# zloyaloha/ray-tracing-practice

Measured on AMD Instinct MI355X. Metric: Msamples/sec (pixels x spp / s), path-traced frame, higher is better.
Workload: dtype f32

## Files before the change

### include/rtp_amd.h

```cpp
#ifndef RTP_AMD_H
#define RTP_AMD_H

#include <stdint.h>

#ifdef __cplusplus
extern "C" {
#endif

typedef enum rt_status {
    RT_OK = 0,
    RT_ERR_INVALID_ARG = 1,
    RT_ERR_NO_DEVICE = 2,
    RT_ERR_HIP = 3,
    RT_ERR_UNSUPPORTED = 4,
    RT_ERR_OUT_OF_MEMORY = 5
} rt_status;


typedef struct rt_vec3 { float e[3]; } rt_vec3;

typedef struct rt_sphere {
    rt_vec3 center;
    float   radius;
    int32_t material_idx;
// ... 107 lines not shown
    int32_t  guard_repack;
    int32_t  kernel;
    uint64_t workspace_bytes;
    int32_t  pass_spp;
    int32_t  stack_levels;
    uint32_t flag_capacity;
    int32_t  scene_in_lds;
    int32_t  lds_treelet;
    int32_t  workgroups_per_cu;
    int32_t  k_inner, k_shade;
    int32_t  reserve_chunk;
    int32_t  reserve_taper;
    int32_t  wavefront_paths;
    int32_t  wavefront_exchange;
    int32_t  wide_nodes;
    int32_t  guard_dynamic_margins;
    int32_t  sphere_only_kernel;
    int32_t  overlap_rework;
    int32_t  primary_visibility;
    int32_t  guard_bail_share;
    int32_t  guard_front_primitives;
    int32_t  reuse_view_lists;
    int32_t  resume_flagged;
} rt_config;


rt_status rt_set_device(int32_t device_ordinal);

rt_status rt_scene_create(const rt_scene_desc *desc, rt_scene **out_scene);

void rt_config_init_sized(rt_config *cfg, uint32_t struct_bytes);
void rt_config_init(rt_config *cfg);
#define rt_config_init(cfg) rt_config_init_sized((cfg), (uint32_t)sizeof(rt_config))
void rt_config_from_env(rt_config *cfg);
rt_status rt_scene_create_ex(const rt_scene_desc *desc, const rt_config *cfg, rt_scene **out_scene);
rt_status rt_scene_set_config(rt_scene *scene, const rt_config *cfg);
rt_status rt_scene_get_config(const rt_scene *scene, rt_config *cfg);

rt_status rt_scene_destroy(rt_scene *scene);

const char *rt_scene_guard_reason(const rt_scene *scene);

int32_t rt_shard_rows(int32_t image_height, const rt_shard *shard);

rt_status rt_render(rt_scene *scene, const rt_camera_data *cam, const rt_shard *shard,
                    float *d_fb_sum, void *hip_stream, int32_t sync, rt_timing *timing);
// ... 144 lines not shown
```

### ray-tracing-practice_amd/csrc/rt_accel.cpp

```cpp
#include "rt_accel.h"
#include "rt_device_math.h"

#include <algorithm>
#include <cmath>
#include <cstdlib>
#include <cstring>
#include <functional>

namespace rtaccel {
namespace {

inline float bits_as_float(int32_t v) { float f; std::memcpy(&f, &v, 4); return f; }

struct LeafRef {
    float box[6];
    int32_t code;
};

struct BuildNode {
    float box[6];
    int32_t child[2];
};

void box_union(const float a[6], const float b[6], float out[6]) {
// ... 479 lines not shown
            out.leaf_boxes.assign(static_cast<size_t>(d.num_spheres) * 8, 0.0f);
            out.plane_leaf_boxes.assign(static_cast<size_t>(d.num_planes) * 8, 0.0f);
            for (LeafRef &l : leaves) {
                const int32_t code = -(l.code + 1);
                const int32_t i = code >> 1;
                float *lb = (code & 1) ? &out.plane_leaf_boxes[static_cast<size_t>(i) * 8] : &out.leaf_boxes[static_cast<size_t>(i) * 8];
                for (int a = 0; a < 6; ++a) lb[a] = l.box[a];
                const double e = (code & 1) ? eps_plane : std::max(eps[static_cast<size_t>(i)], eps_floor);
                const float ef = static_cast<float>(e * (1.0 + 1e-6));
                for (int a = 0; a < 3; ++a) {
                    l.box[2 * a] = std::nextafterf(l.box[2 * a] - ef, -INFINITY);
                    l.box[2 * a + 1] = std::nextafterf(l.box[2 * a + 1] + ef, INFINITY);
                }
            }
            bool derivable = true;
            for (int i = 0; i < d.num_spheres && derivable; ++i) {
                if (leaf_of_sphere[static_cast<size_t>(i)] < 0) continue;
                const rt_sphere &s = d.spheres[i];
                const float *lb = &out.leaf_boxes[static_cast<size_t>(i) * 8];
                for (int a = 0; a < 3; ++a)
                    if (lb[2 * a] != s.center.e[a] - s.radius || lb[2 * a + 1] != s.center.e[a] + s.radius) derivable = false;
            }
            if (derivable && !opt.leaf_table) out.leaf_boxes.clear();
            g.ok = why.empty();
            g.num_front = 0;
            const int front_max = std::min(opt.front_max, kMaxFront);
            while (g.ok && g.num_front < front_max && leaves.size() > 2) {
                float all[6] = {INFINITY, -INFINITY, INFINITY, -INFINITY, INFINITY, -INFINITY};
                size_t big = 0;
                for (size_t k = 0; k < leaves.size(); ++k) {
                    box_union(all, leaves[k].box, all);
                    if (half_area(leaves[k].box) > half_area(leaves[big].box)) big = k;
                }
                if (!(half_area(leaves[big].box) >= 0.5f * half_area(all))) break;
                g.front_code[g.num_front] = -(leaves[big].code + 1);
                std::memcpy(g.front_box[g.num_front], leaves[big].box, sizeof(float) * 6);
                g.num_front++;
                leaves.erase(leaves.begin() + static_cast<std::ptrdiff_t>(big));
            }
            for (int a = 1; a < g.num_front; ++a)
                for (int b = a; b > 0 && (g.front_code[b] & 1) && !(g.front_code[b - 1] & 1); --b) {
                    std::swap(g.front_code[b], g.front_code[b - 1]);
                    for (int k = 0; k < 6; ++k) std::swap(g.front_box[b][k], g.front_box[b - 1][k]);
                }
        }
        g.reason = why;
// ... 315 lines not shown
```

### ray-tracing-practice_amd/csrc/rt_accel.h

```cpp
#pragma once
#include <cstdint>
#include <string>
#include <vector>
#include "../../include/rtp_amd.h"

namespace rtaccel {

constexpr int32_t kTraversalDone = INT32_MIN;

inline int32_t leaf_code(int32_t prim_index, int32_t prim_type) { return -(2 * prim_index + prim_type) - 1; }

constexpr int kMaxFront = 4;

struct Packed {
    std::vector<float> nodes;
    std::vector<float> hnodes;
    std::vector<float> spheres;
    std::vector<int32_t> sphere_mat;
    std::vector<float> planes;
    std::vector<float> materials;
    std::vector<float> tex_data;
    std::vector<int32_t> tex_info;
    std::vector<float> tnodes;
    int32_t num_tnodes = 0;
// ... 3 lines not shown
    int32_t num_internal = 0;
    bool full_pairs = true;
    int32_t num_top_pairs = 0;
    int32_t max_depth = 0;
    std::vector<float> wnodes;
    std::vector<float> whnodes;
    int32_t num_wide = 0, num_top_wide = 0, wroot = kTraversalDone, wide_depth = 0;
    struct Guard {
        bool ok = false;
        std::string reason;
        float center[3] = {0, 0, 0};
        float d0_sq = 0;
        float cluster_radius = 0;
        float box[6] = {0, 0, 0, 0, 0, 0};
        float far_k = 0;
        float dyn_k = 0;
        float dyn_rmax = 0;
        int32_t num_small = 0, num_large = 0;
        float origin_center[3] = {0, 0, 0};
        float origin_radius = 0;
        int32_t num_front = 0;
        int32_t front_code[kMaxFront] = {0, 0, 0, 0};
        float front_box[kMaxFront][6] = {};
    } guard;
    std::vector<float> leaf_boxes;
    std::vector<float> plane_leaf_boxes;
    std::vector<float> guard_leaf_boxes;
    std::vector<int32_t> guard_leaf_codes;
};

enum class TreeMode { Reference, Sah, Guarded, GuardedLeaves };

constexpr float kGuardGammaBound = 24.0f * 5.9604645e-8f;
constexpr float kGuardGammaObserved = 8.0f * 5.9604645e-8f;

struct PackOptions {
    double gamma = kGuardGammaBound;
    bool leaf_table = false;
    int dynamic = 0;
    int front_max = kMaxFront;
    int lds_pair_budget = 0;
};

float half_to_float(uint16_t h);
uint16_t float_to_half_dir(float f, bool toward_minus_inf);

std::string pack_scene(const rt_scene_desc &desc, TreeMode mode, Packed &out, const PackOptions &opt = PackOptions(),
                       const float *camera_hint = nullptr);


struct Magic { uint32_t m, s; };
bool make_magic(uint32_t d, uint64_t n_max, Magic &g);

constexpr uint64_t kWorkIndexLimit = (uint64_t)1 << 30;
constexpr uint64_t kWorkIndexMargin = 64;
constexpr uint64_t kMaxCallPixels = (uint64_t)1 << 24;
constexpr int kMaxPasses = 1024;
constexpr uint64_t kSampleBytes = 12;
constexpr uint64_t kWorkspaceShareOfDevice = 16;

// ... 11 lines not shown
```

### ray-tracing-practice_amd/csrc/rt_capi.hip

```cpp
#include <hip/hip_runtime.h>

#include <cmath>
#include <cstdio>
#include <cstdlib>
#include <cstring>
#include <new>
#include <string>
#include <vector>

#include "../../include/rtp_amd.h"
#include "rt_accel.h"
#include "rt_build.h"
#include "rt_device_math.h"
#include "rt_kernel.hip.inc"
#include "rt_primary.hip.inc"
#include "rt_aov.hip.inc"
#include "rt_adaptive.hip.inc"
#include "rt_nee.hip.inc"
#include "rt_env.hip.inc"
#include "rt_light.hip.inc"

namespace {

thread_local std::string g_last_error;
// ... 47 lines not shown
bool guarded_wanted(const rt_config &cfg, int64_t primitives) {
    if (cfg.traversal == RT_TRAVERSAL_GUARDED) return true;
    return primitives >= cfg.guard_min_primitives;
}

void config_defaults(rt_config &c) {
    std::memset(&c, 0, sizeof(c));
    c.struct_bytes = (uint32_t)sizeof(rt_config);
    c.tree_build = RT_BUILD_HOST_SAH;
    c.guard_gamma_ulps = 0.0f;
    c.traversal = RT_TRAVERSAL_AUTO;
    c.guard_min_primitives = 64;
    c.guard_repack = 1;
    c.kernel = RT_KERNEL_AUTO;
    c.workspace_bytes = 0;
    c.scene_in_lds = 1;
    c.lds_treelet = 1;
    c.reserve_taper = 1;
    c.wide_nodes = 0;
    c.guard_bail_share = 0;
    c.guard_front_primitives = 0;
    c.reuse_view_lists = 0;
    c.resume_flagged = 0;
}

rt_config config_from_caller(const rt_config *in) {
    rt_config c;
    config_defaults(c);
    if (in && in->struct_bytes >= 8) {
        const size_t n = in->struct_bytes < sizeof(rt_config) ? in->struct_bytes : sizeof(rt_config);
        std::memcpy(&c, in, n);
        c.struct_bytes = (uint32_t)sizeof(rt_config);
    }
    if (c.guard_min_primitives < 0) c.guard_min_primitives = 0;
    return c;
}

int32_t lds_pair_budget(const rt_scene_desc &d) {
    bool plain = d.num_planes == 0;
    for (int i = 0; plain && i < d.num_materials; ++i) plain = d.materials[i].texture_id == 0;
    const int64_t budget = (int64_t)kLdsLimit / 2;
    const int64_t lanes = plain ? rtk::kSimpleBlock : rtk::kBlock;
    const int64_t fixed = (int64_t)d.num_spheres * 16 + ((int64_t)d.num_spheres + 3) / 4 * 16 + (int64_t)d.num_planes * 80 +
                          (plain ? 0 : (int64_t)d.num_materials * 16 * RTP_LDS_MAT_ROWS) + 16 * rtk::kConstRows + (lanes / 64) * (8 + 32 * 4) + 7 * lanes * 4;
    const int64_t nodes = (budget - fixed) / rtk::kOctNodeBytes;
    return (int32_t)(nodes < 1 ? 1 : nodes);
}

rtaccel::PackOptions pack_options(const rt_config &cfg, const rt_scene_desc *d = nullptr) {
    rtaccel::PackOptions o;
    if (d && cfg.scene_in_lds != 0) o.lds_pair_budget = lds_pair_budget(*d);
    o.dynamic = cfg.guard_dynamic_margins;
    if (cfg.guard_gamma_ulps > 0.0f) o.gamma = (double)cfg.guard_gamma_ulps * 5.9604644775390625e-8;
    o.leaf_table = cfg.guard_exact_leaf_table != 0;
    o.front_max = cfg.guard_front_primitives < 0 ? 0 : rtaccel::kMaxFront;
    return o;
}
uint32_t bail_share_of(const rt_config &cfg) {
    if (cfg.guard_bail_share < 0) return 0u;
    const uint32_t s = cfg.guard_bail_share == 0 ? kDefaultBailShare : (uint32_t)cfg.guard_bail_share;
    return s > 255u ? 255u : s;
}
uint32_t bail_floor() {
    static const uint32_t f = [] { const int v = env_int("RTP_BAIL_FLOOR", (int)kDefaultBailFloor); return (uint32_t)(v < 0 ? 0 : v > 255 ? 255 : v); }();
    return f;
}
uint32_t bail_latest() {
    static const uint32_t f = [] { const int v = env_int("RTP_BAIL_LATEST", (int)kDefaultBailLatest); return (uint32_t)(v < 1 ? 1 : v > 8 ? 8 : v); }();
    return f;
}
template <class T>
void copy_out(const T &src, T *dst, uint32_t caller_bytes) {
    const uint32_t n = caller_bytes < sizeof(T) ? caller_bytes : (uint32_t)sizeof(T);
    std::memcpy(dst, &src, n);
    dst->struct_bytes = n;
}
rt_status timing_check(const rt_timing *t) {
    if (t && t->struct_bytes < 8) { g_last_error = "rt_timing.struct_bytes is not set (rt_timing_init)"; return RT_ERR_INVALID_ARG; }
// ... 50 lines not shown
    int4 *tex_info = nullptr;
    uint32_t *queue = nullptr;
    float *slab = nullptr;
    size_t slab_floats = 0;
    rtaccel::Packed::Guard guard;
    std::vector<rt_sphere> host_spheres;
    std::vector<rt_plane> host_planes;
    std::vector<rt_bvh_node> host_nodes;
    bool device_built = false;
    int repacks = 0;
    bool repack_refused = false;
    bool guard_paused = false;
    struct Feedback {
        uint32_t *host = nullptr; hipEvent_t start = nullptr, done = nullptr;
        bool pending = false, guarded = false, exploring = false;
        int passes = 0; uint64_t samples = 0, serial = 0;
    };
    Feedback feedback[kFeedbackSlots];
    int feedback_next = 0;
    double guarded_ns_per_sample = 0.0, exact_ns_per_sample = 0.0;
    bool explore_exact = false;
    uint64_t frame_serial = 0;
    uint32_t trip_test = 0;
    const uint32_t *last_traced_pixels = nullptr;
    int32_t last_spp = 0;
    float4 *leaf_boxes = nullptr, *plane_leaf_boxes = nullptr;
    uint32_t *flag_list = nullptr;
    uint32_t *resume_tag = nullptr; float4 *resume_state = nullptr;
    size_t flag_cap = 0;
    uint32_t *dirty = nullptr, *dirty_list = nullptr;
    size_t dirty_cap = 0;
    hipStream_t aux_stream = nullptr, list_stream = nullptr;
    hipEvent_t ev_fork = nullptr, ev_join = nullptr, ev_listed = nullptr;
    uint32_t *cand = nullptr;
    size_t cand_pixels = 0;
    struct CandKey { float view[12]; int32_t dims[9]; int repacks; hipStream_t stream; bool valid = false; } cand_key;
    int32_t num_internal = 0, num_spheres = 0, num_planes = 0, num_materials = 0, root = rtk::kDone, tree_depth = 0;
    CallClock clock[kNumClocks];
    std::vector<hipEvent_t> pass_events;
    int timed_passes = 0;
    rt_timing last{};
    int last_passes = 0;
    uint64_t last_samples = 0;
    bool timed = false;
    int num_cus = 0;
    uint64_t device_bytes = 0;
// ... 70 lines not shown
        if (shard && shard->num_parts > 1) return fail(RT_ERR_INVALID_ARG, "a tile and a shard in one call");
        if (tile->w <= 0 || tile->h <= 0 || tile->x0 < 0 || tile->y0 < 0 || (int64_t)tile->x0 + tile->w > cam->image_width ||
            (int64_t)tile->y0 + tile->h > cam->image_height)
            return fail(RT_ERR_INVALID_ARG, "tile outside the image");
        P.local_rows = tile->h;
        P.row_w = tile->w;
        P.tile_x0 = tile->x0;
        P.tile_y0 = tile->y0;
    }
    P.nodes = sc->nodes; P.hnodes = sc->hnodes; P.num_internal = sc->num_internal; P.root = sc->root;
    P.whnodes = sc->whnodes; P.wroot = sc->wroot;
    P.tnodes = sc->tnodes; P.num_tnodes = sc->num_tnodes;
    P.xnodes = sc->xnodes; P.num_top = sc->num_top;
    P.spheres = sc->spheres; P.num_spheres = sc->num_spheres;
    P.planes = sc->planes; P.num_planes = sc->num_planes;
    P.materials = sc->materials; P.num_materials = sc->num_materials;
    P.sphere_mat = sc->sphere_mat;
    P.tex_data = sc->tex_data; P.tex_info = sc->tex_info;
    P.queue = sc->queue;
    if ((uint64_t)P.local_rows * (uint64_t)P.row_w > (1u << 24)) return fail(RT_ERR_UNSUPPORTED, "more than 2^24 pixels per call");
    P.total_work = 0;
    P.stats = sc->queue + kQueueStats;
    P.trip_test = sc->trip_test;
    {
        const uint64_t pixels = (uint64_t)P.local_rows * (uint64_t)P.row_w;
        if (!make_magic((uint32_t)P.row_w, pixels + 1, P.magic_width) ||
            !make_magic((uint32_t)P.band_rows, (uint64_t)P.local_rows + 1, P.magic_band))
            return fail(RT_ERR_UNSUPPORTED, "image too large for the work index arithmetic");
    }
    P.stack_levels = 0;
    P.leaf_boxes = sc->leaf_boxes;
    P.plane_leaf_boxes = sc->plane_leaf_boxes;
    std::memcpy(P.g_center, sc->guard.center, 12);
    P.g_d0sq = sc->guard.d0_sq;
    P.g_rs = sc->guard.cluster_radius;
    P.g_fark = sc->guard.far_k;
    P.g_dynk = sc->guard.dyn_k;
    {
        const double sk = std::sqrt((double)sc->guard.dyn_k * (double)rtk::kDynSlack) * (1.0 + 4e-6);
        P.g_dyn_sqrtk = std::nextafterf((float)sk, INFINITY);
        P.g_dyn_b = std::nextafterf((float)(sk * 1.7320508075688772 * (double)sc->guard.dyn_rmax * (1.0 + 1e-6)), INFINITY);
        P.g_dyn_c3 = std::nextafterf((float)(sk * 1.7320508075688772), INFINITY);
        P.g_dyn_kslack = std::nextafterf((float)((double)sc->guard.dyn_k * (double)rtk::kDynSlack), INFINITY);
    }
    P.num_front = sc->guard.num_front;
    std::memcpy(P.front_code, sc->guard.front_code, sizeof(P.front_code));
    std::memcpy(P.front_box, sc->guard.front_box, sizeof(P.front_box));
    std::memcpy(P.g_box, sc->guard.box, 24);
    P.k_inner = sc->cfg.k_inner > 0 ? sc->cfg.k_inner : 24;
    P.k_shade = sc->cfg.k_shade > 0 ? sc->cfg.k_shade : 48;
    P.chunk = 64u;
    return RT_OK;
}

rt_status repack_for_camera(rt_scene *sc, const float cam[3], hipStream_t stream) {
// ... 93 lines not shown
    cfg->guard_keep = env_int("RTP_GUARD_KEEP", cfg->guard_keep);
    if (env_int("RTP_NO_REPACK", 0)) cfg->guard_repack = 0;
    if (const char *v = getenv("RTP_SLAB_GIB")) { const double g = atof(v); if (g > 0) cfg->workspace_bytes = (uint64_t)(g * 1073741824.0); }
    cfg->pass_spp = env_int("RTP_PASS_SPP", cfg->pass_spp);
    cfg->stack_levels = env_int("RTP_STACK_LEVELS", cfg->stack_levels);
    cfg->flag_capacity = (uint32_t)env_int("RTP_FLAG_CAP", (int)cfg->flag_capacity);
    if (env_int("RTP_NO_LDS_SCENE", 0)) cfg->scene_in_lds = 0;
    if (env_int("RTP_NO_TREELET", 0)) cfg->lds_treelet = 0;
    cfg->workgroups_per_cu = env_int("RTP_WGS_PER_CU", cfg->workgroups_per_cu);
    cfg->k_inner = env_int("RTP_K_INNER", cfg->k_inner);
    cfg->k_shade = env_int("RTP_K_SHADE", cfg->k_shade);
    cfg->reserve_chunk = env_int("RTP_CHUNK", cfg->reserve_chunk);
    cfg->wavefront_paths = env_int("RTP_WF_PATHS", cfg->wavefront_paths);
    cfg->wavefront_exchange = env_int("RTP_WF_EXCHANGE", cfg->wavefront_exchange);
    if (env_int("RTP_NO_TAPER", 0)) cfg->reserve_taper = 0;
    cfg->wide_nodes = env_int("RTP_WIDE", cfg->wide_nodes);
    if (env_int("RTP_NO_SIMPLE", 0)) cfg->sphere_only_kernel = -1;
    if (env_int("RTP_NO_OVERLAP", 0)) cfg->overlap_rework = -1;
    if (env_int("RTP_NO_PRIMARY", 0)) cfg->primary_visibility = -1;
    cfg->guard_bail_share = env_int("RTP_BAIL_SHARE", cfg->guard_bail_share);
    if (env_int("RTP_NO_FRONT", 0)) cfg->guard_front_primitives = -1;
    if (env_int("RTP_NO_VIEW_CACHE", 0)) cfg->reuse_view_lists = -1;
    if (env_int("RTP_NO_RESUME", 0)) cfg->resume_flagged = -1;
    copy_out(full, user, user->struct_bytes);
}

rt_status rt_scene_create(const rt_scene_desc *desc, rt_scene **out_scene) { return rt_scene_create_ex(desc, nullptr, out_scene); }

rt_status rt_scene_set_config(rt_scene *sc, const rt_config *cfg) {
    if (!sc || !cfg) return fail(RT_ERR_INVALID_ARG, "null argument");
    rt_config c = config_from_caller(cfg);
    c.tree_build = sc->cfg.tree_build;
    c.guard_gamma_ulps = sc->cfg.guard_gamma_ulps;
    c.guard_exact_leaf_table = sc->cfg.guard_exact_leaf_table;
    c.guard_dynamic_margins = sc->cfg.guard_dynamic_margins;
    c.guard_front_primitives = sc->cfg.guard_front_primitives;
    sc->cfg = c;
    return RT_OK;
}

rt_status rt_scene_get_config(const rt_scene *sc, rt_config *cfg) {
    if (!sc || !cfg) return fail(RT_ERR_INVALID_ARG, "null argument");
    if (cfg->struct_bytes < 8) return fail(RT_ERR_INVALID_ARG, "rt_config.struct_bytes is not set (rt_config_init)");
    copy_out(sc->cfg, cfg, cfg->struct_bytes);
    return RT_OK;
}

rt_status rt_scene_create_ex(const rt_scene_desc *desc, const rt_config *user_cfg, rt_scene **out_scene) {
    if (!desc || !out_scene) return fail(RT_ERR_INVALID_ARG, "null argument");
    *out_scene = nullptr;
    const rt_config cfg = config_from_caller(user_cfg);
    if (cfg.guard_gamma_ulps < 0.0f || !(cfg.guard_gamma_ulps == cfg.guard_gamma_ulps)) return fail(RT_ERR_INVALID_ARG, "guard_gamma_ulps must be >= 0");
    rtaccel::Packed pk;
    const rtaccel::PackOptions popt = pack_options(cfg, desc);
    const bool device_build = cfg.tree_build == RT_BUILD_DEVICE_LBVH;
    std::string err = rtaccel::pack_scene(*desc, device_build ? rtaccel::TreeMode::GuardedLeaves : rtaccel::TreeMode::Guarded, pk, popt);
    if (!err.empty()) return fail(RT_ERR_INVALID_ARG, err);
    if (device_build && !pk.guard.ok) {
        err = rtaccel::pack_scene(*desc, rtaccel::TreeMode::Guarded, pk, popt);
// ... 52 lines not shown
        sc->host_nodes.assign(desc->nodes, desc->nodes + desc->num_nodes);
        sc->device_built = device_build;
    }
    if (hipMalloc((void **)&sc->queue, kQueueWords * 4) != hipSuccess) return bail(fail(RT_ERR_OUT_OF_MEMORY, "hipMalloc(queue) failed"));
    if (sc->clock[kClockRender].make() != RT_OK) return bail(fail(RT_ERR_HIP, "hipEventCreate failed"));
    sc->num_internal = pk.num_internal;
    sc->num_top_pairs = pk.num_top_pairs;
    sc->num_spheres = (int32_t)pk.sphere_mat.size();
    sc->num_planes = (int32_t)(pk.planes.size() / 20);
    sc->num_materials = (int32_t)(pk.materials.size() / 12);
    sc->root = pk.root;
    sc->tree_depth = pk.max_depth;
    *out_scene = sc;
    return RT_OK;
}

rt_status rt_scene_destroy(rt_scene *sc) {
    if (!sc) return RT_OK;
    (void)hipFree(sc->tnodes);
    (void)hipFree(sc->xnodes);
    (void)hipFree(sc->nodes); (void)hipFree(sc->hnodes); (void)hipFree(sc->whnodes);
    (void)hipFree(sc->spheres); (void)hipFree(sc->planes); (void)hipFree(sc->materials);
    (void)hipFree(sc->sphere_mat); (void)hipFree(sc->tex_data); (void)hipFree(sc->tex_info); (void)hipFree(sc->queue); (void)hipFree(sc->slab);
    (void)hipFree(sc->leaf_boxes); (void)hipFree(sc->plane_leaf_boxes); (void)hipFree(sc->flag_list);
    (void)hipFree(sc->dirty); (void)hipFree(sc->dirty_list); (void)hipFree(sc->cand);
    (void)hipFree(sc->resume_tag); (void)hipFree(sc->resume_state);
    if (sc->aux_stream) (void)hipStreamDestroy(sc->aux_stream);
    if (sc->list_stream) (void)hipStreamDestroy(sc->list_stream);
    if (sc->ev_listed) (void)hipEventDestroy(sc->ev_listed);
    if (sc->ev_fork) (void)hipEventDestroy(sc->ev_fork);
    if (sc->ev_join) (void)hipEventDestroy(sc->ev_join);
    for (hipEvent_t e : sc->pass_events) (void)hipEventDestroy(e);
    for (hipEvent_t e : sc->aov_events) (void)hipEventDestroy(e);
    for (CallClock &c : sc->clock) c.destroy();
    (void)hipFree(sc->adapt_mom); (void)hipFree(sc->adapt_list); (void)hipFree(sc->adapt_work); (void)hipFree(sc->adapt_counters);
    (void)hipFree(sc->nee_index_dev); (void)hipFree(sc->nee_cdf_dev); (void)hipFree(sc->nee_pmf_dev);
    for (rt_scene::Feedback &f : sc->feedback) {
        if (f.done) { if (f.pending) (void)hipEventSynchronize(f.done); (void)hipEventDestroy(f.done); }
        if (f.start) (void)hipEventDestroy(f.start);
        if (f.host) (void)hipHostFree(f.host);
    }
    delete sc;
    return RT_OK;
}

const char *rt_scene_guard_reason(const rt_scene *sc) {
    if (!sc) return "null scene";
// ... 1746 lines not shown
    const std::string err = rtbuild::build_lbvh(boxes, codes, n, tree);
    if (!err.empty()) return fail(RT_ERR_HIP, "device BVH build: " + err);
    info[0] = tree.root; info[1] = tree.num_internal; info[2] = tree.depth; info[3] = 0;
    hipError_t e = hipSuccess;
    if (tree.num_internal < 0 || tree.num_internal > n - 1) {
        (void)hipFree(tree.nodes); (void)hipFree(tree.hnodes);
        return fail(RT_ERR_HIP, "device BVH build: " + std::to_string(tree.num_internal) + " records for " + std::to_string(n) + " leaves");
    }
    if (tree.num_internal > 0) {
        e = hipMemcpy(nodes_out, tree.nodes, 64 * (size_t)tree.num_internal, hipMemcpyDeviceToHost);
        if (e == hipSuccess) e = hipMemcpy(hnodes_out, tree.hnodes, 32 * (size_t)tree.num_internal, hipMemcpyDeviceToHost);
    }
    (void)hipFree(tree.nodes); (void)hipFree(tree.hnodes);
    HIP_TRY(e);
    return RT_OK;
}

rt_status rt_debug_trip_test(rt_scene *sc, uint32_t on) {
    if (!sc) return fail(RT_ERR_INVALID_ARG, "null argument");
    sc->trip_test = on;
    return RT_OK;
}

rt_status rt_debug_read_stats(rt_scene *sc, uint32_t out[16]) {
    if (!sc || !out) return fail(RT_ERR_INVALID_ARG, "null argument");
    HIP_TRY(hipDeviceSynchronize());
    HIP_TRY(hipMemcpy(out, sc->queue + kQueueStats, 60, hipMemcpyDeviceToHost));
    return RT_OK;
}

#endif

rt_status rt_last_kernel_ms(rt_scene *sc, float *ms) {
    if (!sc || !ms) return fail(RT_ERR_INVALID_ARG, "null argument");
    *ms = 0.0f;
    if (!sc->timed) return RT_OK;
    return sc->clock[kClockRender].elapsed(*ms);
}

rt_status rt_render_to_host(rt_scene *sc, const rt_camera_data *cam, const rt_shard *shard, float *h_fb_sum, rt_timing *timing) {
    if (!sc || !cam || !h_fb_sum) return fail(RT_ERR_INVALID_ARG, "null argument");
    const int32_t rows = rt_shard_rows(cam->image_height, shard);
    const size_t bytes = (size_t)rows * (size_t)(cam->image_width > 0 ? cam->image_width : 0) * 3 * sizeof(float);
    if (bytes == 0) return RT_OK;
    float *d_fb = nullptr;
    Scratch mem;
// ... 97 lines not shown
```

### ray-tracing-practice_amd/csrc/rt_kernel.hip.inc

```
#pragma once

namespace rtk {

using namespace rtd;

constexpr int kWave = 64;
constexpr int32_t kDone = INT32_MIN;
#ifndef RTP_BLOCK
#define RTP_BLOCK 768
#endif
#ifndef RTP_MIN_WAVES
#define RTP_MIN_WAVES 6
#endif
#ifndef RTP_UNROLL
#define RTP_UNROLL 4
#endif
#ifndef RTP_LDS_MAT_ROWS
#define RTP_LDS_MAT_ROWS 1
#endif
#ifndef RTP_UNROLL_WIDE
#define RTP_UNROLL_WIDE 3
#endif
#ifndef RTP_TRIPWIRE
#ifdef RTP_DEV_BUILD
// ... 27 lines not shown
    int32_t row_w, tile_x0, tile_y0;
    const float4 *nodes;     int32_t num_internal; int32_t root;
    const float4 *hnodes;
    const float4 *whnodes;   int32_t wroot;
    const float4 *tnodes;    int32_t num_tnodes;
    const float4 *xnodes;    int32_t num_top;
    const float4 *spheres;   int32_t num_spheres;
    const float4 *planes;    int32_t num_planes;
    const float4 *materials; int32_t num_materials;
    const int32_t *sphere_mat;
    const float4 *tex_data;  const int4 *tex_info;
    float *fb;
    float *slab;
    uint32_t slab_pitch;
    uint32_t num_pixels;
    int32_t pass_first, pass_count;
    Magic magic_count, magic_width, magic_band;
    uint32_t *queue;
    uint32_t chunk;
    uint32_t taper_shift;
    uint32_t full_chunk, full_taper;
    uint32_t *stats;
    uint32_t trip_test;
    uint32_t total_work;
    int32_t stack_levels;
    int32_t k_inner, k_shade;
    const float4 *leaf_boxes;
    const float4 *plane_leaf_boxes;
    float g_center[3]; float g_d0sq, g_rs, g_fark; float g_box[6];
    float g_dynk;
    float g_dyn_sqrtk, g_dyn_b;
    float g_dyn_c3, g_dyn_kslack;
    int32_t num_front; int32_t front_code[4]; float front_box[4 * 6];
    uint32_t *flag_list; uint32_t *flag_count; uint32_t flag_cap;
    uint32_t *abandon; uint32_t bail_share; uint32_t bail_floor, bail_latest;
    uint32_t flag_chunk_words;
    uint32_t *resume_tag; float4 *resume_state; uint32_t resume_shift;
    uint32_t *dirty; uint32_t *dirty_list; uint32_t *dirty_count;
    const uint32_t *work_list; const uint32_t *work_count; uint32_t work_cap;
    uint32_t consts[14 * 4];
    const uint32_t *cand;
    const uint32_t *order;
    const uint32_t *traced_pixels;
    const int32_t *probe_ijs; float *probe_rad; int32_t *probe_rays; uint32_t *probe_seed; int32_t probe_n;
};

struct Lane {
    f3 o, d, inv;
    float closest;
    int32_t hit;
    int32_t node;
    int32_t sp;
    int32_t pend;
    float e;
    uint32_t seed;
    f3 beta, color;
    int32_t depth;
};

__device__ __forceinline__ f3 ld3(const float *p) { return mk(p[0], p[1], p[2]); }
__device__ __forceinline__ int32_t as_int(float f) { return __float_as_int(f); }

template <bool kClamp = false>
__device__ __forceinline__ void begin_ray(Lane &L, f3 o, f3 d, int32_t root) {
    L.o = o;
    L.d = d;
#if RTP_FAST_RCP_SQRT && defined(__HIP_DEVICE_COMPILE__)
    L.inv = mk(recip_estimate(d.x), recip_estimate(d.y), recip_estimate(d.z));
    if (__builtin_expect(!(recip_in_fence(d.x) && recip_in_fence(d.y) && recip_in_fence(d.z)), 0)) L.inv = mk(1.0f / d.x, 1.0f / d.y, 1.0f / d.z);
#else
    L.inv = mk(1.0f / d.x, 1.0f / d.y, 1.0f / d.z);
#endif
    if (kClamp) L.inv = mk(__builtin_amdgcn_fmed3f(L.inv.x, -1e18f, 1e18f), __builtin_amdgcn_fmed3f(L.inv.y, -1e18f, 1e18f), __builtin_amdgcn_fmed3f(L.inv.z, -1e18f, 1e18f));
    L.closest = 1e30f;
    L.hit = -1;
    L.node = root;
    L.sp = 0;
    L.pend = 0;
}

constexpr int32_t kLevelBytes = kWave * 4;
template <bool kSent = false>
__device__ __forceinline__ void pop(Lane &L, const uint32_t *stack) {
    if (kSent) {
        L.sp -= kLevelBytes;
        L.node = (int32_t)*reinterpret_cast<const uint32_t *>(reinterpret_cast<const char *>(stack) + L.sp);
    } else if (L.sp > 0) {
        L.sp--;
        L.node = (int32_t)stack[L.sp * kWave];
    } else {
        L.node = kDone;
    }
}

__device__ __forceinline__ f3 inv_exact(const Lane &L) {
// ... 515 lines not shown
    const float4 t00 = d[y0w * W + x0w], t10 = d[y0w * W + x1], t01 = d[y1 * W + x0w], t11 = d[y1 * W + x1];
    const f3 top = add(scale(1.0f - dx, mk(t00.x, t00.y, t00.z)), scale(dx, mk(t10.x, t10.y, t10.z)));
    const f3 bot = add(scale(1.0f - dx, mk(t01.x, t01.y, t01.z)), scale(dx, mk(t11.x, t11.y, t11.z)));
    return add(scale(1.0f - dy, top), scale(dy, bot));
}

template <bool kSimple = false, bool kClamped = false, class SphereTab>
__device__ __forceinline__ bool guard_final_check(const Lane &L, const KParams &P, SphereTab spheres) {
    const int32_t code = L.hit;
    const int32_t idx = code >> 1;
    float enter;
    bool in;
    if (!kSimple && ((code & 1) || P.leaf_boxes)) {
        const float4 *tab = (code & 1) ? P.plane_leaf_boxes : P.leaf_boxes;
        const float4 B0 = tab[2 * idx], B1 = tab[2 * idx + 1];
        in = slab<kClamped>(L, B0.x, B0.z, B1.x, B0.y, B0.w, B1.y, 1e30f, enter);
    } else {
        const float4 sp = spheres[idx];
        in = slab<kClamped>(L, sp.x - sp.w, sp.y - sp.w, sp.z - sp.w, sp.x + sp.w, sp.y + sp.w, sp.z + sp.w, 1e30f, enter);
    }
    return in && (L.closest > enter);
}

__device__ __forceinline__ f3 scatter_diffuse_dir(f3 in_sphere, f3 normal) {
    const f3 u = unit(in_sphere);
    f3 dir = dot(u, normal) > 0.0f ? u : neg(u);
    if (near_zero(dir)) dir = normal;
    return dir;
}

template <bool kGuard = false, int kMatStride = 3, bool kSimple = false, bool kPrim = false, bool kClamped = false, class SphereTab, class PlaneTab, class MatTab, class IdxTab>
__device__ __forceinline__ bool shade(Lane &L, const KParams &P, SphereTab spheres, PlaneTab planes, MatTab materials,
                                      IdxTab sphere_mat, f3 &out_o, f3 &out_d) {
    if (kGuard && (L.depth & kFlagBit)) return false;
    if (L.hit < 0) {
        L.color = add(L.color, mul(L.beta, mk(P.bg[0], P.bg[1], P.bg[2])));
        return false;
    }
    const int32_t code = L.hit;
    const int32_t idx = code >> 1;
    const float t = L.closest;
    const bool checked = kPrim && (L.depth & kFreshBit) != 0;
    if (kPrim) L.depth &= ~kFreshBit;
    if (kGuard && !(checked | guard_final_check<kSimple, kClamped>(L, P, spheres))) {
        L.depth |= kFlagBit | RTP_WHY(2);
        return false;
    }
    const f3 point = add(L.o, scale(t, L.d));
    f3 normal;
    bool front;
    int32_t mat_idx;
    float tu = 0.0f, tv = 0.0f;
    const bool is_plane = !kSimple && (code & 1) != 0;
    f3 outward = mk(0, 0, 0);
    if (is_plane) {
        const float4 P0 = planes[5 * idx + 0];
        const float4 P2 = planes[5 * idx + 2];
        outward = mk(P0.x, P0.y, P0.z);
        mat_idx = as_int(P2.w);
    } else {
        const float4 s = spheres[idx];
        outward = divs(sub(point, mk(s.x, s.y, s.z)), s.w);
        mat_idx = sphere_mat[idx];
    }
    front = dot(L.d, outward) < 0;
    normal = front ? outward : neg(outward);

    const float4 MA = materials[kMatStride * mat_idx + 0];
    const float4 ME = kMatStride >= 2 ? materials[kMatStride * mat_idx + 1] : P.materials[3 * mat_idx + 1];
    const int32_t type = as_int(MA.w) & 3;
    const int32_t tex_id = kSimple ? 0 : (as_int(MA.w) >> 2);
    f3 albedo = mk(MA.x, MA.y, MA.z);
    if (tex_id != 0) {
        if (is_plane) {
            const float4 P1 = planes[5 * idx + 1];
            const float4 P2 = planes[5 * idx + 2];
            const float4 P3 = planes[5 * idx + 3];
            const float4 P4 = planes[5 * idx + 4];
            const f3 ph = sub(point, mk(P4.x, P4.y, P4.z));
            const f3 w = mk(P1.x, P1.y, P1.z);
            tu = dot(w, cross(ph, mk(P3.x, P3.y, P3.z)));
            tv = dot(w, cross(mk(P2.x, P2.y, P2.z), ph));
        } else {
            const float theta = acos_libm(outward.y);
// ... 647 lines not shown
```

### ray-tracing-practice_amd/csrc/rt_primary.hip.inc

```
#pragma once
#include "rt_beam.h"

namespace rtk {

constexpr int kCandWords = 16;
constexpr uint32_t kCandNone = 0xffffffffu;

__global__ void __launch_bounds__(256) cand_kernel(const KParams P, uint32_t *cand, double coord_max) {
    const uint32_t q = blockIdx.x * 256u + threadIdx.x;
    if (q >= P.num_pixels) return;
    const uint32_t pjl = q / (uint32_t)P.row_w;
    const int32_t pi = (int32_t)(q - pjl * (uint32_t)P.row_w) + P.tile_x0;
    int32_t pj = (int32_t)pjl + P.tile_y0;
    if (P.num_parts != 1) {
        const uint32_t band = pjl / (uint32_t)P.band_rows;
        pj = (int32_t)((band * (uint32_t)P.num_parts + (uint32_t)P.part) * (uint32_t)P.band_rows + (pjl - band * (uint32_t)P.band_rows));
    }
    const rtbeam::Beam beam = rtbeam::make_beam(P.origin, P.p00, P.du, P.dv, pi, pj, coord_max);
    uint32_t codes[kCandWords - 1];
    const float *tab = reinterpret_cast<const float *>(P.nodes);
    int n = rtbeam::beam_candidates(beam, [tab](int32_t k) { return tab + (size_t)k * 16; }, P.root, (double)P.g_dynk, codes, kCandWords - 1);
    n = rtbeam::beam_front_candidates(beam, P.num_front, P.front_code, P.front_box, (double)P.g_dynk, codes, n, kCandWords - 1);
    uint32_t *out = cand + (size_t)q * kCandWords;
    out[0] = n < 0 ? kCandNone : (uint32_t)n;
// ... 100 lines not shown
    return L.hit >= 0 ? L.hit : kPrimMiss;
}
template <bool kPlanes>
__device__ __forceinline__ int32_t test_lane_list(Lane &L, const KParams &P, uint32_t q, float4 &hs) {
    const uint32_t *list = P.cand + (size_t)q * kCandWords;
    const uint32_t n = list[0];
    if (n == kCandNone) return kPrimWalk;
    const RayConst rc = ray_const(L);
    for (uint32_t c = 0; c < n; ++c) {
        const uint32_t code = list[1 + c];
        const int32_t idx = (int32_t)(code >> 1);
        if (kPlanes && (code & 1u)) test_plane<true>(L, P.planes, idx, (int32_t)code);
        else {
            const float4 sp = P.spheres[idx];
            test_sphere_ray<true, true>(L, sp, (int32_t)code, rc.a, rc.da, rc.y);
            if (L.hit == (int32_t)code) hs = sp;
        }
    }
    return L.hit >= 0 ? L.hit : kPrimMiss;
}
template <bool kPlanes>
__device__ __forceinline__ void finish_primary(Lane &L, const KParams &P, int32_t code_out, uint32_t seed1, float4 hs, float *rec) {
    if (P.leaf_boxes == nullptr) {
        float enter;
        const bool in = slab(L, hs.x - hs.w, hs.y - hs.w, hs.z - hs.w, hs.x + hs.w, hs.y + hs.w, hs.z + hs.w, 1e30f, enter);
        const bool sphere_hit = code_out >= 0 && (!kPlanes || !(code_out & 1));
        if (sphere_hit && !(in && L.closest > enter)) L.depth |= kFlagBit;
        if (kPlanes && code_out >= 0 && (code_out & 1) && !guard_final_check<false>(L, P, P.spheres)) L.depth |= kFlagBit;
    } else if (code_out >= 0 && !guard_final_check<false>(L, P, P.spheres)) {
        L.depth |= kFlagBit;
    }
    if (L.depth & kFlagBit) code_out = kPrimFlag;
    rec[0] = L.closest;
    rec[1] = __int_as_float(code_out);
    rec[2] = __uint_as_float(seed1);
}

template <bool kPlanes>
__global__ void __launch_bounds__(256) primary_kernel(const KParams P) {
    const uint32_t lane = threadIdx.x & 63u;
    const uint32_t wave = (blockIdx.x * 256u + threadIdx.x) >> 6, num_waves = gridDim.x * 4u;
    const uint32_t batches = (P.total_work + 63u) >> 6;
    for (uint32_t b = wave; b < batches; b += num_waves) {
        const uint32_t w = b * 64u + lane;
        if (w >= P.total_work) continue;
        int32_t pi, pj;
        uint32_t k, record;
        map_work<false>(P, w, pi, pj, k, 0u, nullptr, nullptr, &record);
        const uint32_t q = P.pass_count == 64 ? (w >> 6) : div_magic(w, P.magic_count);
        if (P.cand[(size_t)q * kCandWords] == 0u) continue;
        Lane L;
        f3 ray_o, ray_d;
        const uint32_t seed1 = sample_seed1(wang_hash((uint32_t)pi * (uint32_t)P.width + (uint32_t)pj), P.pass_first + (int32_t)k);
        camera_ray<false>(L, P, pi, pj, seed1, ray_o, ray_d);
        begin_ray(L, ray_o, ray_d, 0);
        const uint32_t q0 = __builtin_amdgcn_readfirstlane(q);
        float4 hs = make_float4(0.0f, 0.0f, 0.0f, 0.0f);
        const int32_t code_out = __ballot(q != q0) == 0ull ? test_uniform_list<kPlanes>(L, P, q0, hs) : test_lane_list<kPlanes>(L, P, q, hs);
        finish_primary<kPlanes>(L, P, code_out, seed1, hs, P.slab + (size_t)record * 3);
    }
}

template <bool kPlanes>
__global__ void __launch_bounds__(256) primary_pixel_kernel(const KParams P) {
    const uint32_t lane = threadIdx.x & 63u;
    const uint32_t wave = __builtin_amdgcn_readfirstlane((blockIdx.x * 256u + threadIdx.x) >> 6), num_waves = gridDim.x * 4u;
    for (uint32_t q = wave; q < P.num_pixels; q += num_waves) {
        const uint32_t pjl = div_magic(q, P.magic_width);
        const int32_t pi = (int32_t)(q - pjl * (uint32_t)P.row_w) + P.tile_x0;
        int32_t pj = (int32_t)pjl + P.tile_y0;
        if (P.num_parts != 1) {
            const uint32_t band = div_magic(pjl, P.magic_band);
            pj = (int32_t)((band * (uint32_t)P.num_parts + (uint32_t)P.part) * (uint32_t)P.band_rows + (pjl - band * (uint32_t)P.band_rows));
        }
        float *row = P.slab + (size_t)q * P.slab_pitch * 3;
        if (*(k_u32 *)(uintptr_t)(P.cand + (size_t)q * kCandWords) == 0u) continue;
        const uint32_t base_seed = wang_hash((uint32_t)pi * (uint32_t)P.width + (uint32_t)pj);
        for (uint32_t k = lane; k < (uint32_t)P.pass_count; k += 64u) {
            Lane L;
            f3 ray_o, ray_d;
            const uint32_t seed1 = sample_seed1(base_seed, P.pass_first + (int32_t)k);
            camera_ray<false>(L, P, pi, pj, seed1, ray_o, ray_d);
            begin_ray(L, ray_o, ray_d, 0);
            float4 hs = make_float4(0.0f, 0.0f, 0.0f, 0.0f);
            const int32_t code_out = test_uniform_list<kPlanes>(L, P, q, hs);
            finish_primary<kPlanes>(L, P, code_out, seed1, hs, row + (size_t)k * 3);
        }
    }
}

}
```

### ray-tracing-practice_amd/rtp_bindings.py

```python
import ctypes as C
import os

import numpy as np

_HERE = os.path.dirname(os.path.abspath(__file__))


class Vec3(C.Structure):
    _fields_ = [("e", C.c_float * 3)]


class Sphere(C.Structure):
    _fields_ = [("center", Vec3), ("radius", C.c_float), ("material_idx", C.c_int32), ("_pad", C.c_int32 * 3)]


class Plane(C.Structure):
    _fields_ = [("type", C.c_int32), ("D", C.c_float), ("material_idx", C.c_int32), ("w", Vec3), ("u", Vec3),
                ("v", Vec3), ("base", Vec3), ("normal", Vec3), ("_pad", C.c_int32 * 2)]


class Material(C.Structure):
    _fields_ = [("type", C.c_int32), ("fuzz", C.c_float), ("ir", C.c_float), ("absorption", Vec3), ("albedo", Vec3),
                ("emit", Vec3), ("texture_id", C.c_uint64), ("reserved", C.c_uint64)]

# ... 222 lines not shown
        self.close()

    def __del__(self):
        try:
            self.close()
        except Exception:
            pass


TRAVERSAL_AUTO, TRAVERSAL_EXACT, TRAVERSAL_GUARDED = 0, 1, 2
BUILD_HOST_SAH, BUILD_DEVICE_LBVH = 0, 1
KERNEL_AUTO, KERNEL_MEGA, KERNEL_WAVEFRONT = 0, 1, 2


class Config(C.Structure):
    _fields_ = [("struct_bytes", C.c_uint32), ("tree_build", C.c_int32), ("guard_gamma_ulps", C.c_float),
                ("guard_exact_leaf_table", C.c_int32), ("traversal", C.c_int32), ("guard_min_primitives", C.c_int32),
                ("guard_keep", C.c_int32), ("guard_repack", C.c_int32), ("kernel", C.c_int32), ("workspace_bytes", C.c_uint64),
                ("pass_spp", C.c_int32), ("stack_levels", C.c_int32), ("flag_capacity", C.c_uint32), ("scene_in_lds", C.c_int32),
                ("lds_treelet", C.c_int32), ("workgroups_per_cu", C.c_int32), ("k_inner", C.c_int32), ("k_shade", C.c_int32),
                ("reserve_chunk", C.c_int32), ("reserve_taper", C.c_int32), ("wavefront_paths", C.c_int32),
                ("wavefront_exchange", C.c_int32), ("wide_nodes", C.c_int32), ("guard_dynamic_margins", C.c_int32),
                ("sphere_only_kernel", C.c_int32), ("overlap_rework", C.c_int32), ("primary_visibility", C.c_int32),
                ("guard_bail_share", C.c_int32), ("guard_front_primitives", C.c_int32), ("reuse_view_lists", C.c_int32), ("resume_flagged", C.c_int32)]


def new_config():
    cfg = Config()
    lib = amd_lib()
    if hasattr(lib, "rt_config_init_sized"):
        lib.rt_config_init_sized(C.byref(cfg), C.sizeof(Config))
        assert cfg.struct_bytes == C.sizeof(Config) or os.environ.get("RTP_AMD_LIB"), (cfg.struct_bytes, C.sizeof(Config))
    else:
        assert os.environ.get("RTP_AMD_LIB")
        lib.rt_config_init(C.byref(cfg))
    return cfg


class ConfigInfo(C.Structure):
    _fields_ = [("num_frames", C.c_int32), ("width", C.c_int32), ("height", C.c_int32), ("max_depth", C.c_int32),
                ("sqrt_spp", C.c_int32), ("fov_degrees", C.c_float)]


assert C.sizeof(Sphere) == 32 and C.sizeof(Plane) == 80 and C.sizeof(Material) == 64
assert C.sizeof(BvhNode) == 36 and C.sizeof(CameraData) == 76

RTP_AMD_SYMBOLS = [
# ... 819 lines not shown
```

Before: 11990.

## Skip primary-hit leaf-box slab check when hit point is provably inside box

Adds a host-side analysis that marks scenes where a cheap error-bounded interior test on the hit point is enough to certify a sphere hit lies inside its leaf box. In the primary-visibility kernel, the slab test and the ray reciprocal are now computed only when some lane in the wavefront is unsure or hit a plane. begin_ray skips computing inv for primary rays. The aim is to cut per-sample ALU work in finish_primary, at the cost of extra host checks, a new config flag, and a debug counter path.

```diff
diff --git a/include/rtp_amd.h b/include/rtp_amd.h
--- a/include/rtp_amd.h
+++ b/include/rtp_amd.h
@@ -153,6 +153,7 @@
     int32_t  guard_front_primitives;
     int32_t  reuse_view_lists;
     int32_t  resume_flagged;
+    int32_t  leafbox_filter;
 } rt_config;
 
 
diff --git a/ray-tracing-practice_amd/csrc/rt_accel.cpp b/ray-tracing-practice_amd/csrc/rt_accel.cpp
--- a/ray-tracing-practice_amd/csrc/rt_accel.cpp
+++ b/ray-tracing-practice_amd/csrc/rt_accel.cpp
@@ -525,6 +525,18 @@
                     if (lb[2 * a] != s.center.e[a] - s.radius || lb[2 * a + 1] != s.center.e[a] + s.radius) derivable = false;
             }
             if (derivable && !opt.leaf_table) out.leaf_boxes.clear();
+            g.leaf_sure = opt.leaf_sure && out.leaf_boxes.empty();
+            double extent = 0;
+            for (int i = 0; i < d.num_spheres; ++i) {
+                if (leaf_of_sphere[static_cast<size_t>(i)] < 0 || (g.num_small > 0 && large[static_cast<size_t>(i)])) continue;
+                const rt_sphere &s = d.spheres[i];
+                for (int a = 0; a < 3; ++a) extent = std::max(extent, std::fabs(double(s.center.e[a])) + s.radius);
+            }
+            for (int i = 0; i < d.num_spheres && g.leaf_sure; ++i) {
+                if (leaf_of_sphere[static_cast<size_t>(i)] < 0) continue;
+                const double r = d.spheres[i].radius;
+                if (!(r >= kLeafSureRMin && r <= kLeafSureRMax) || !((4.0 * extent + r) / r <= kLeafSureMaxRatio)) g.leaf_sure = false;
+            }
             g.ok = why.empty();
             g.num_front = 0;
             const int front_max = std::min(opt.front_max, kMaxFront);
diff --git a/ray-tracing-practice_amd/csrc/rt_accel.h b/ray-tracing-practice_amd/csrc/rt_accel.h
--- a/ray-tracing-practice_amd/csrc/rt_accel.h
+++ b/ray-tracing-practice_amd/csrc/rt_accel.h
@@ -49,6 +49,7 @@
         int32_t num_front = 0;
         int32_t front_code[kMaxFront] = {0, 0, 0, 0};
         float front_box[kMaxFront][6] = {};
+        bool leaf_sure = false;
     } guard;
     std::vector<float> leaf_boxes;
     std::vector<float> plane_leaf_boxes;
@@ -61,8 +62,16 @@
 constexpr float kGuardGammaBound = 24.0f * 5.9604645e-8f;
 constexpr float kGuardGammaObserved = 8.0f * 5.9604645e-8f;
 
+constexpr int kLeafSureKappaLog2 = -21;
+constexpr float kLeafSureKappa = 1.0f / (float)(1 << -kLeafSureKappaLog2);
+constexpr float kLeafSureTMax = 1099511627776.0f;
+constexpr float kLeafSureRMin = 8.673617379884035e-19f;
+constexpr float kLeafSureRMax = 1152921504606846976.0f;
+constexpr double kLeafSureMaxRatio = 2730.0;
+
 struct PackOptions {
     double gamma = kGuardGammaBound;
+    bool leaf_sure = true;
     bool leaf_table = false;
     int dynamic = 0;
     int front_max = kMaxFront;
diff --git a/ray-tracing-practice_amd/csrc/rt_capi.hip b/ray-tracing-practice_amd/csrc/rt_capi.hip
--- a/ray-tracing-practice_amd/csrc/rt_capi.hip
+++ b/ray-tracing-practice_amd/csrc/rt_capi.hip
@@ -93,6 +93,7 @@
     c.guard_front_primitives = 0;
     c.reuse_view_lists = 0;
     c.resume_flagged = 0;
+    c.leafbox_filter = 0;
 }
 
 rt_config config_from_caller(const rt_config *in) {
@@ -125,6 +126,7 @@
     if (cfg.guard_gamma_ulps > 0.0f) o.gamma = (double)cfg.guard_gamma_ulps * 5.9604644775390625e-8;
     o.leaf_table = cfg.guard_exact_leaf_table != 0;
     o.front_max = cfg.guard_front_primitives < 0 ? 0 : rtaccel::kMaxFront;
+    o.leaf_sure = cfg.leafbox_filter >= 0;
     return o;
 }
 uint32_t bail_share_of(const rt_config &cfg) {
@@ -221,6 +223,7 @@
     bool explore_exact = false;
     uint64_t frame_serial = 0;
     uint32_t trip_test = 0;
+    unsigned long long *leaf_count = nullptr; bool leaf_count_on = false;
     const uint32_t *last_traced_pixels = nullptr;
     int32_t last_spp = 0;
     float4 *leaf_boxes = nullptr, *plane_leaf_boxes = nullptr;
@@ -337,6 +340,7 @@
     P.total_work = 0;
     P.stats = sc->queue + kQueueStats;
     P.trip_test = sc->trip_test;
+    P.leaf_count = sc->leaf_count_on ? sc->leaf_count : nullptr;
     {
         const uint64_t pixels = (uint64_t)P.local_rows * (uint64_t)P.row_w;
         if (!make_magic((uint32_t)P.row_w, pixels + 1, P.magic_width) ||
@@ -346,6 +350,7 @@
     P.stack_levels = 0;
     P.leaf_boxes = sc->leaf_boxes;
     P.plane_leaf_boxes = sc->plane_leaf_boxes;
+    P.leaf_sure = sc->guard.leaf_sure && sc->leaf_boxes == nullptr ? 1u : 0u;
     std::memcpy(P.g_center, sc->guard.center, 12);
     P.g_d0sq = sc->guard.d0_sq;
     P.g_rs = sc->guard.cluster_radius;
@@ -485,6 +490,7 @@
     if (env_int("RTP_NO_FRONT", 0)) cfg->guard_front_primitives = -1;
     if (env_int("RTP_NO_VIEW_CACHE", 0)) cfg->reuse_view_lists = -1;
     if (env_int("RTP_NO_RESUME", 0)) cfg->resume_flagged = -1;
+    if (env_int("RTP_NO_LEAFBOX_FILTER", 0)) cfg->leafbox_filter = -1;
     copy_out(full, user, user->struct_bytes);
 }
 
@@ -498,6 +504,7 @@
     c.guard_exact_leaf_table = sc->cfg.guard_exact_leaf_table;
     c.guard_dynamic_margins = sc->cfg.guard_dynamic_margins;
     c.guard_front_primitives = sc->cfg.guard_front_primitives;
+    c.leafbox_filter = sc->cfg.leafbox_filter;
     sc->cfg = c;
     return RT_OK;
 }
@@ -596,7 +603,7 @@
     (void)hipFree(sc->nodes); (void)hipFree(sc->hnodes); (void)hipFree(sc->whnodes);
     (void)hipFree(sc->spheres); (void)hipFree(sc->planes); (void)hipFree(sc->materials);
     (void)hipFree(sc->sphere_mat); (void)hipFree(sc->tex_data); (void)hipFree(sc->tex_info); (void)hipFree(sc->queue); (void)hipFree(sc->slab);
-    (void)hipFree(sc->leaf_boxes); (void)hipFree(sc->plane_leaf_boxes); (void)hipFree(sc->flag_list);
+    (void)hipFree(sc->leaf_boxes); (void)hipFree(sc->plane_leaf_boxes); (void)hipFree(sc->flag_list); (void)hipFree(sc->leaf_count);
     (void)hipFree(sc->dirty); (void)hipFree(sc->dirty_list); (void)hipFree(sc->cand);
     (void)hipFree(sc->resume_tag); (void)hipFree(sc->resume_state);
     if (sc->aux_stream) (void)hipStreamDestroy(sc->aux_stream);
@@ -2389,6 +2396,22 @@
     return RT_OK;
 }
 
+rt_status rt_debug_leafbox_count(rt_scene *sc, int32_t arm, uint64_t out[4]) {
+    if (!sc || (!arm && !out)) return fail(RT_ERR_INVALID_ARG, "null argument");
+    HIP_TRY(hipDeviceSynchronize());
+    if (arm) {
+        if (!sc->leaf_count) HIP_TRY(hipMalloc((void **)&sc->leaf_count, 24));
+        HIP_TRY(hipMemset(sc->leaf_count, 0, 24));
+        sc->leaf_count_on = true;
+        return RT_OK;
+    }
+    sc->leaf_count_on = false;
+    if (!sc->leaf_count) return fail(RT_ERR_INVALID_ARG, "rt_debug_leafbox_count: never armed");
+    HIP_TRY(hipMemcpy(out, sc->leaf_count, 24, hipMemcpyDeviceToHost));
+    out[3] = sc->guard.leaf_sure && sc->leaf_boxes == nullptr ? 1u : 0u;
+    return RT_OK;
+}
+
 rt_status rt_debug_read_stats(rt_scene *sc, uint32_t out[16]) {
     if (!sc || !out) return fail(RT_ERR_INVALID_ARG, "null argument");
     HIP_TRY(hipDeviceSynchronize());
diff --git a/ray-tracing-practice_amd/csrc/rt_kernel.hip.inc b/ray-tracing-practice_amd/csrc/rt_kernel.hip.inc
--- a/ray-tracing-practice_amd/csrc/rt_kernel.hip.inc
+++ b/ray-tracing-practice_amd/csrc/rt_kernel.hip.inc
@@ -73,11 +73,13 @@
     uint32_t full_chunk, full_taper;
     uint32_t *stats;
     uint32_t trip_test;
+    unsigned long long *leaf_count;
     uint32_t total_work;
     int32_t stack_levels;
     int32_t k_inner, k_shade;
     const float4 *leaf_boxes;
     const float4 *plane_leaf_boxes;
+    uint32_t leaf_sure;
     float g_center[3]; float g_d0sq, g_rs, g_fark; float g_box[6];
     float g_dynk;
     float g_dyn_sqrtk, g_dyn_b;
@@ -112,16 +114,20 @@
 __device__ __forceinline__ f3 ld3(const float *p) { return mk(p[0], p[1], p[2]); }
 __device__ __forceinline__ int32_t as_int(float f) { return __float_as_int(f); }
 
-template <bool kClamp = false>
+__device__ __forceinline__ f3 ray_inv(f3 d) {
+#if RTP_FAST_RCP_SQRT && defined(__HIP_DEVICE_COMPILE__)
+    f3 inv = mk(recip_estimate(d.x), recip_estimate(d.y), recip_estimate(d.z));
+    if (__builtin_expect(!(recip_in_fence(d.x) && recip_in_fence(d.y) && recip_in_fence(d.z)), 0)) inv = mk(1.0f / d.x, 1.0f / d.y, 1.0f / d.z);
+    return inv;
+#else
+    return mk(1.0f / d.x, 1.0f / d.y, 1.0f / d.z);
+#endif
+}
+template <bool kClamp = false, bool kInv = true>
 __device__ __forceinline__ void begin_ray(Lane &L, f3 o, f3 d, int32_t root) {
     L.o = o;
     L.d = d;
-#if RTP_FAST_RCP_SQRT && defined(__HIP_DEVICE_COMPILE__)
-    L.inv = mk(recip_estimate(d.x), recip_estimate(d.y), recip_estimate(d.z));
-    if (__builtin_expect(!(recip_in_fence(d.x) && recip_in_fence(d.y) && recip_in_fence(d.z)), 0)) L.inv = mk(1.0f / d.x, 1.0f / d.y, 1.0f / d.z);
-#else
-    L.inv = mk(1.0f / d.x, 1.0f / d.y, 1.0f / d.z);
-#endif
+    if (kInv) L.inv = ray_inv(d);
     if (kClamp) L.inv = mk(__builtin_amdgcn_fmed3f(L.inv.x, -1e18f, 1e18f), __builtin_amdgcn_fmed3f(L.inv.y, -1e18f, 1e18f), __builtin_amdgcn_fmed3f(L.inv.z, -1e18f, 1e18f));
     L.closest = 1e30f;
     L.hit = -1;
@@ -683,6 +689,16 @@
     return in && (L.closest > enter);
 }
 
+constexpr float kLeafSureKappa = rtaccel::kLeafSureKappa;
+__device__ __forceinline__ bool leaf_sure(f3 o, f3 pt, float t, float4 s) {
+    const float mx = s.w - fabsf(pt.x - s.x), my = s.w - fabsf(pt.y - s.y), mz = s.w - fabsf(pt.z - s.z);
+    const float sx = __builtin_fmaf(2.0f, fabsf(pt.x), (fabsf(o.x) + fabsf(s.x)) + s.w);
+    const float sy = __builtin_fmaf(2.0f, fabsf(pt.y), (fabsf(o.y) + fabsf(s.y)) + s.w);
+    const float sz = __builtin_fmaf(2.0f, fabsf(pt.z), (fabsf(o.z) + fabsf(s.z)) + s.w);
+    const bool inside = __builtin_fmaf(-kLeafSureKappa, sx, mx) > 0.0f && __builtin_fmaf(-kLeafSureKappa, sy, my) > 0.0f && __builtin_fmaf(-kLeafSureKappa, sz, mz) > 0.0f;
+    return inside && t > 0.001f && t < rtaccel::kLeafSureTMax;
+}
+
 __device__ __forceinline__ f3 scatter_diffuse_dir(f3 in_sphere, f3 normal) {
     const f3 u = unit(in_sphere);
     f3 dir = dot(u, normal) > 0.0f ? u : neg(u);
@@ -721,6 +737,18 @@
         mat_idx = as_int(P2.w);
     } else {
         const float4 s = spheres[idx];
+#ifdef RTP_DEV_BUILD
+        if (!kGuard && P.leaf_count != nullptr && P.leaf_boxes == nullptr) {
+            const bool sure = leaf_sure(L.o, point, t, s);
+            const bool exact = guard_final_check<true, kClamped>(L, P, spheres);
+            const uint64_t all = __ballot(true), unsure = __ballot(!sure), bad = __ballot(sure && !exact);
+            if ((all & ((1ull << __lane_id()) - 1ull)) == 0ull) {
+                atomicAdd(P.leaf_count + 0, (unsigned long long)__popcll(all));
+                if (unsure) atomicAdd(P.leaf_count + 1, (unsigned long long)__popcll(unsure));
+                if (bad) atomicAdd(P.leaf_count + 2, (unsigned long long)__popcll(bad));
+            }
+        }
+#endif
         outward = divs(sub(point, mk(s.x, s.y, s.z)), s.w);
         mat_idx = sphere_mat[idx];
     }
diff --git a/ray-tracing-practice_amd/csrc/rt_primary.hip.inc b/ray-tracing-practice_amd/csrc/rt_primary.hip.inc
--- a/ray-tracing-practice_amd/csrc/rt_primary.hip.inc
+++ b/ray-tracing-practice_amd/csrc/rt_primary.hip.inc
@@ -146,13 +146,20 @@
 template <bool kPlanes>
 __device__ __forceinline__ void finish_primary(Lane &L, const KParams &P, int32_t code_out, uint32_t seed1, float4 hs, float *rec) {
     if (P.leaf_boxes == nullptr) {
-        float enter;
-        const bool in = slab(L, hs.x - hs.w, hs.y - hs.w, hs.z - hs.w, hs.x + hs.w, hs.y + hs.w, hs.z + hs.w, 1e30f, enter);
         const bool sphere_hit = code_out >= 0 && (!kPlanes || !(code_out & 1));
-        if (sphere_hit && !(in && L.closest > enter)) L.depth |= kFlagBit;
-        if (kPlanes && code_out >= 0 && (code_out & 1) && !guard_final_check<false>(L, P, P.spheres)) L.depth |= kFlagBit;
-    } else if (code_out >= 0 && !guard_final_check<false>(L, P, P.spheres)) {
-        L.depth |= kFlagBit;
+        const bool plane_hit = kPlanes && code_out >= 0 && (code_out & 1);
+        bool unsure = sphere_hit;
+        if (P.leaf_sure) unsure = sphere_hit && !leaf_sure(L.o, add(L.o, scale(L.closest, L.d)), L.closest, hs);
+        if (__any(unsure || plane_hit)) {
+            L.inv = ray_inv(L.d);
+            float enter;
+            const bool in = slab(L, hs.x - hs.w, hs.y - hs.w, hs.z - hs.w, hs.x + hs.w, hs.y + hs.w, hs.z + hs.w, 1e30f, enter);
+            if (sphere_hit && !(in && L.closest > enter)) L.depth |= kFlagBit;
+            if (plane_hit && !guard_final_check<false>(L, P, P.spheres)) L.depth |= kFlagBit;
+        }
+    } else if (__any(code_out >= 0)) {
+        L.inv = ray_inv(L.d);
+        if (code_out >= 0 && !guard_final_check<false>(L, P, P.spheres)) L.depth |= kFlagBit;
     }
     if (L.depth & kFlagBit) code_out = kPrimFlag;
     rec[0] = L.closest;
@@ -177,7 +184,7 @@
         f3 ray_o, ray_d;
         const uint32_t seed1 = sample_seed1(wang_hash((uint32_t)pi * (uint32_t)P.width + (uint32_t)pj), P.pass_first + (int32_t)k);
         camera_ray<false>(L, P, pi, pj, seed1, ray_o, ray_d);
-        begin_ray(L, ray_o, ray_d, 0);
+        begin_ray<false, false>(L, ray_o, ray_d, 0);
         const uint32_t q0 = __builtin_amdgcn_readfirstlane(q);
         float4 hs = make_float4(0.0f, 0.0f, 0.0f, 0.0f);
         const int32_t code_out = __ballot(q != q0) == 0ull ? test_uniform_list<kPlanes>(L, P, q0, hs) : test_lane_list<kPlanes>(L, P, q, hs);
@@ -205,7 +212,7 @@
             f3 ray_o, ray_d;
             const uint32_t seed1 = sample_seed1(base_seed, P.pass_first + (int32_t)k);
             camera_ray<false>(L, P, pi, pj, seed1, ray_o, ray_d);
-            begin_ray(L, ray_o, ray_d, 0);
+            begin_ray<false, false>(L, ray_o, ray_d, 0);
             float4 hs = make_float4(0.0f, 0.0f, 0.0f, 0.0f);
             const int32_t code_out = test_uniform_list<kPlanes>(L, P, q, hs);
             finish_primary<kPlanes>(L, P, code_out, seed1, hs, row + (size_t)k * 3);
diff --git a/ray-tracing-practice_amd/rtp_bindings.py b/ray-tracing-practice_amd/rtp_bindings.py
--- a/ray-tracing-practice_amd/rtp_bindings.py
+++ b/ray-tracing-practice_amd/rtp_bindings.py
@@ -268,7 +268,8 @@
                 ("reserve_chunk", C.c_int32), ("reserve_taper", C.c_int32), ("wavefront_paths", C.c_int32),
                 ("wavefront_exchange", C.c_int32), ("wide_nodes", C.c_int32), ("guard_dynamic_margins", C.c_int32),
                 ("sphere_only_kernel", C.c_int32), ("overlap_rework", C.c_int32), ("primary_visibility", C.c_int32),
-                ("guard_bail_share", C.c_int32), ("guard_front_primitives", C.c_int32), ("reuse_view_lists", C.c_int32), ("resume_flagged", C.c_int32)]
+                ("guard_bail_share", C.c_int32), ("guard_front_primitives", C.c_int32), ("reuse_view_lists", C.c_int32), ("resume_flagged", C.c_int32),
+                ("leafbox_filter", C.c_int32)]
 
 
 def new_config():
```

Result: no change. 12050 (median of 6 runs) (+0.5%).
